# zcash/halo2

Measured on NVIDIA H100. Metric: msm_pairs_per_s, higher is better.
Workload: dtype u32x8 (255-bit modular integers)

## Files before the change

### halo2_b200/csrc/capi_msm.cu

```cuda
#define H2_MSM_QUAD_ACCUM_REFS (g_ctx.small_accum_refs)
#include "util_kernels.cuh"
#include "msm.cuh"
#include "ipa.cuh"
#include "ntt.cuh"
#include "ecfft.cuh"
#include "fixedbase.cuh"

struct PassBases { const affine *bases; uint32_t c = 0, mode = 0; uint64_t stride = 0; };
static PassBases pass_bases(const BaseSet *b) {
    if (b->dtable.p) return {b->dtable.as<affine>(), H2_FB_BITS, 2, b->n};
    if (b->table.p) return {b->table.as<affine>(), b->c, 1, b->n};
    return {b->buf.as<affine>()};
}


static int exclusive_scan_u32(uint32_t *d, uint64_t n, cudaStream_t s, const uint32_t *only_if = nullptr) {
    const uint64_t per_block = (uint64_t)H2_SCAN_BLOCK * H2_SCAN_ITEMS;
    uint32_t nb = (uint32_t)((n + per_block - 1) / per_block);
    if (g_ctx.scan_blocks.ensure((size_t)nb * 4 + 16)) return 1;
    uint32_t *bs = g_ctx.scan_blocks.as<uint32_t>();
    LAUNCH(scan_block_sums_kernel, nb, H2_SCAN_BLOCK, 0, s, d, n, bs, only_if);
    LAUNCH(scan_single_block_kernel, 1, H2_SCAN_BLOCK, 0, s, bs, nb, only_if);
    LAUNCH(scan_apply_kernel, nb, H2_SCAN_BLOCK, 0, s, d, n, bs, only_if);
    return 0;
// ... 108 lines not shown
        return msm_issue_or_replay(issue, !bc, d_scalars, d_bases, d_out, n, stride, H2_FB_BITS, fp.sets, scalars_mont, out_canonical, fast, s);
    }
    const uint32_t glv = (!fixed && X.glv_on && n < (1ull << 30)) ? 1u : 0u;
    if (c == 0) c = X.window_override ? X.window_override : msm_default_window(n, glv);
    if (c > 24) return fail("msm: window bits > 24");
    const uint32_t K = (bc && !fixed && bc->k > 1) ? bc->k : 1u;
    const uint32_t force_cap = X.sort_bins ? 0u : H2_MSM_NO_BINS;
    MsmPlan p;
    msm_make_plan(p, n, c, 0, 0, fixed, stride, glv, sets, force_cap);
    p.chunks = K;
    p.fast = (fixed == 1 && !bc && fast && p.cap != 0) ? 1u : 0u;
    if (ran_fast) *ran_fast = p.fast != 0;
    if (p.fast && p.T < p.cap) { p.T = p.cap; p.acc_chunk[0] = p.T; }
    p.natural = (p.fast && p.G <= X.natural_max_buckets && p.max_refs <= 2 * H2_MSM_QUAD_ACCUM_REFS && (X.accum_ways <= 1 || X.accum_ways >= 12)) ? 1u : 0u;
    MsmPlan pk[H2_MAX_UPLOAD_CHUNKS];
    size_t first[H2_MAX_UPLOAD_CHUNKS + 1];
    for (uint32_t j = 0; j <= K; j++) first[j] = chunk_first(n, K, j);
    uint64_t ref_space = 0, max_items = 0, part_total = 0;
    uint32_t t_max = 0;
    for (uint32_t j = 0; j < K; j++) {
        if (K == 1) pk[0] = p;
        else msm_make_plan(pk[j], first[j + 1] - first[j], c, 0, 0, fixed, stride, glv, sets, force_cap);
        if (pk[j].ref_space >= (1ull << 32)) return fail("msm: n * windows exceeds 2^32 references");
        ref_space = pk[j].ref_space > ref_space ? pk[j].ref_space : ref_space;
        max_items = pk[j].max_items > max_items ? pk[j].max_items : max_items;
        part_total = pk[j].part_total > part_total ? pk[j].part_total : part_total;
        t_max = pk[j].T > t_max ? pk[j].T : t_max;
    }
    bool thread_per_item = false;
    for (uint32_t j = 0; j < K; j++) thread_per_item |= pk[j].max_refs > (pk[j].fixed ? 2 : 1) * H2_MSM_QUAD_ACCUM_REFS;
    record(fixed, c, p.W, p.sets, thread_per_item ? 1u : 0u, p.natural, p.fast);
    uint64_t ba_space = 0;
    if (!fixed && X.ba_rounds) {
        size_t free_b = 0, total_b = 0;
        CU(cudaMemGetInfo(&free_b, &total_b));
        for (uint32_t j = 0; j < K; j++) {
            if (pk[j].max_refs > H2_MSM_QUAD_ACCUM_REFS && (uint64_t)K * pk[j].ref_space * 56 <= free_b / 2) msm_plan_ba(pk[j], X.ba_rounds, X.ba_target);
            if (pk[j].ba) ba_space = pk[j].ref_space > ba_space ? pk[j].ref_space : ba_space;
        }
    }
    if (K == 1) p.ba = pk[0].ba;
    if (ba_space)
        for (uint32_t r = 0; r < H2_BA_MAX_ROUNDS; r++)
            if (X.ba_lv[r].ensure(K * ((ba_space >> (r + 1)) + 1) * sizeof(affine))) return 1;
    if (glv && (X.bases_phi.ensure(n * sizeof(affine)) || X.glv_parts.ensure(n * 32))) return 1;
    if (fixed && (uint64_t)p.W * stride >= (1ull << 31)) return fail("msm: window table too large for 31-bit references");
    if (p.G >= (1ull << 32) || n >= (1ull << 31)) return fail("msm: n * windows exceeds 2^32 references");
    if (scalars_mont && X.scal_canon.ensure(n * p.sets * sizeof(fe))) return 1;
    const size_t small_words = 2 * (t_max + 2) + 8;
    part_total += 1;
    if (X.counts.ensure(K * (p.G + 1) * 4) || X.cursor.ensure(K * 2 * p.G * 4) || X.refs.ensure(K * ref_space * 4) ||
        X.size_hist.ensure(K * small_words * 4) || X.items.ensure(K * max_items * sizeof(uint2)) ||
        X.bucket_sum.ensure(K * p.G * sizeof(xyzz)) || X.pkey.ensure(K * part_total * 4) || X.pstart.ensure(K * part_total * 4) ||
        X.pend.ensure(K * part_total * 4) || X.ppt.ensure(K * part_total * sizeof(xyzz)) ||
        X.ra_t.ensure((size_t)p.Wb * p.m1 * sizeof(xyzz)) || X.ra_e.ensure((size_t)p.Wb * p.m1 * sizeof(xyzz)) ||
        X.r0.ensure((size_t)p.Wb * p.nb0 * H2_R0_ROWS * sizeof(xyzz)) || X.r1.ensure((size_t)p.Wb * p.r1_rows * sizeof(xyzz)) ||
        X.wsum.ensure((size_t)p.Wb * sizeof(xyzz)))
        return 1;
    MsmBuffers Mk[H2_MAX_UPLOAD_CHUNKS];
    for (uint32_t j = 0; j < K; j++) {
        MsmBuffers &M = Mk[j];
        const size_t o = first[j];
        M.scalars = d_scalars + o; M.bases = d_bases + o; M.bases_phi = X.bases_phi.as<affine>() + o;
        M.glv_parts = X.glv_parts.as<uint32_t>() + 8 * o; M.scalars_mont = scalars_mont ? 1u : 0u;
        M.scal_canon = X.scal_canon.as<fe>() + o;
        M.counts = X.counts.as<uint32_t>() + j * (p.G + 1); M.cursor = X.cursor.as<uint32_t>() + j * 2 * p.G; M.cursor2 = M.cursor + p.G;
        M.refs = X.refs.as<uint32_t>() + j * ref_space;
        M.size_hist = X.size_hist.as<uint32_t>() + j * small_words; M.size_cursor = M.size_hist + (pk[j].T + 2); M.flags = M.size_cursor + (pk[j].T + 2);
        M.items = X.items.as<uint2>() + j * max_items;
        M.bucket_sum = X.bucket_sum.as<xyzz>() + j * p.G;
        for (uint32_t r = 0; r < H2_BA_MAX_ROUNDS; r++) M.ba[r] = ba_space ? X.ba_lv[r].as<affine>() + j * ((ba_space >> (r + 1)) + 1) : nullptr;
        M.pkey = X.pkey.as<uint32_t>() + j * part_total; M.pstart = X.pstart.as<uint32_t>() + j * part_total;
        M.pend = X.pend.as<uint32_t>() + j * part_total; M.ppt = X.ppt.as<xyzz>() + j * part_total;
        M.ra_t = X.ra_t.as<xyzz>(); M.ra_e = X.ra_e.as<xyzz>(); M.r0 = X.r0.as<xyzz>(); M.r1 = X.r1.as<xyzz>();
        M.wsum = X.wsum.as<xyzz>(); M.result = d_out;
    }
    X.last_flags = Mk[0].flags;

    {
        const uint64_t per_block = (uint64_t)H2_SCAN_BLOCK * H2_SCAN_ITEMS;
        if (X.scan_blocks.ensure((size_t)((p.G + 1 + per_block - 1) / per_block) * 4 + 16)) return 1;
    }
    issue = [&]() -> int {
        if (!p.fast) CU(cudaMemsetAsync(X.counts.p, 0, K * (p.G + 1) * 4, s));
        CU(cudaMemsetAsync(X.cursor.p, 0, K * 2 * p.G * 4, s));
        CU(cudaMemsetAsync(X.size_hist.p, 0, K * small_words * 4, s));
        CU(cudaMemsetAsync(X.bucket_sum.p, 0, K * p.G * sizeof(xyzz), s));
        if (!p.fast) CU(cudaMemsetAsync(X.pkey.p, 0xff, K * part_total * 4, s));

        auto k_bin = msm_bin_kernel<P, PS>;
        auto k_hist = msm_hist_kernel<P, PS>;
        auto k_scatter = msm_scatter_kernel<P, PS>;
        auto k_ihist = msm_item_hist_kernel<P, PS>;
        auto k_ibases = msm_item_bases_kernel<P, PS>;
        auto k_iplace = msm_item_place_kernel<P, PS>;
        auto k_accum0 = msm_accum0_kernel<P, PS>;
        auto k_accum0q = msm_accum0_quad_kernel<P, PS>;
        auto k_accum0p2 = msm_accum0_pair_kernel<P, PS>;
        auto k_accum0s2 = msm_accum0_split_kernel<P, PS, 2>;
        auto k_accum0s4 = msm_accum0_split_kernel<P, PS, 4>;
        auto k_accum0m2 = msm_accum0_multi_kernel<P, PS, 2>;
        auto k_accum0m4 = msm_accum0_multi_kernel<P, PS, 4>;
        auto k_ba = X.ba_variant == 1 ? msm_ba_round_kernel<P, PS, 4, 5> : X.ba_variant == 2 ? msm_ba_round_kernel<P, PS, 2, 4>
                  : X.ba_variant == 3 ? msm_ba_round_kernel<P, PS, 2, 5> : msm_ba_round_kernel<P, PS, 4, 4>;
        auto k_accum0p = msm_accum0_pts_kernel<P, PS>;
        auto k_accumN = msm_accumN_kernel<P, PS>;
        auto k_rest = msm_accum_rest_kernel<P, PS>;
        auto k_reduceA = msm_reduceA_kernel<P, PS>;
        auto k_r0 = msm_r0_kernel<P, PS>;
        auto k_r1 = msm_r1_kernel<P, PS>;
        auto k_wsum = msm_wsum_kernel<P, PS>;
        auto k_final = msm_final_kernel<P, PS>;
        for (uint32_t j = 0; j < K; j++) {
            const MsmPlan &q = pk[j];
            const MsmBuffers &M = Mk[j];
            if (bc && bc->k) {
                for (uint32_t e = (K > 1 ? j : 0); e < (K > 1 ? j + 1 : bc->k); e++) {
                    if (bc->wait_recorded(2 * e + 1)) return fail("msm: the upload of the inputs failed");
                    CU(cudaStreamWaitEvent(s, bc->ev_scal[e], 0));
                }
            }
            if (q.cap == 0) CU(cudaMemsetAsync(M.flags + 1, 0x01, 4, s));
            else LAUNCH(k_bin, blocks_for(q.n * q.sets, 256), 256, 0, s, q, M);
            if (!q.fast) {
                LAUNCH(k_hist, blocks_for(q.n * q.sets, 256), 256, 0, s, q, M);
                if (exclusive_scan_u32(M.counts, q.G + 1, s, M.flags + 1)) return 1;
                LAUNCH(k_scatter, blocks_for(q.n * q.sets, 256), 256, 0, s, q, M);
            }
            if (!q.natural) {
                LAUNCH(k_ihist, blocks_for(q.G, 256), 256, 0, s, q, M);
                LAUNCH(k_ibases, 1, 32, 0, s, q, M);
                LAUNCH(k_iplace, blocks_for(q.G, 256), 256, 0, s, q, M);
            }
            if (bc && bc->k) {
                for (uint32_t e = (K > 1 ? j : 0); e < (K > 1 ? j + 1 : bc->k); e++) {
                    if (bc->wait_recorded(2 * e + 2)) return fail("msm: the upload of the inputs failed");
                    CU(cudaStreamWaitEvent(s, bc->ev[e], 0));
                }
            }
            if (q.glv) {
                auto k_phi = msm_phi_kernel<P, PS>;
                LAUNCH(k_phi, blocks_for(q.n, 256), 256, 0, s, M.bases, M.bases_phi, (uint64_t)q.n);
            }
            prof_begin(PROF_MSM_ACCUM0, s);
            if (q.max_refs <= (q.fixed ? 2 : 1) * H2_MSM_QUAD_ACCUM_REFS) {
                if (X.accum_ways == 4) LAUNCH(k_accum0m4, blocks_for(q.max_items * 16, 128), 128, 0, s, q, M);
                else if (X.accum_ways == 2) LAUNCH(k_accum0m2, blocks_for(q.max_items * 8, 128), 128, 0, s, q, M);
                else if (X.accum_ways == 0) LAUNCH(k_accum0p2, blocks_for(q.max_items * 2, 128), 128, 0, s, q, M);
                else if (X.accum_ways == 12) LAUNCH(k_accum0s2, blocks_for(q.max_items * 2, 128), 128, 0, s, q, M);
                else if (X.accum_ways == 14) LAUNCH(k_accum0s4, blocks_for(q.max_items * 4, 128), 128, 0, s, q, M);
                else LAUNCH(k_accum0q, blocks_for(q.max_items * 4, 128), 128, 0, s, q, M);
            }
            else {
                for (uint32_t r = 1; r <= q.ba; r++)
                    LAUNCH(k_ba, blocks_for((q.max_items + q.ba_m[r - 1] - 1) / q.ba_m[r - 1], 128), 128, 0, s, q, M, r);
                if (q.ba) LAUNCH(k_accum0p, blocks_for(q.max_items, 128), 128, 0, s, q, M);
                LAUNCH(k_accum0, blocks_for(q.max_items, 128), 128, 0, s, q, M);
            }
            prof_end(s);
            if (!q.fast) {
                if (q.acc_levels > 1) LAUNCH(k_accumN, blocks_for(q.acc_threads[1], 128), 128, 0, s, q, M, 1u);
                if (q.acc_levels > 2) LAUNCH(k_accumN, blocks_for(q.acc_threads[2], 128), 128, 0, s, q, M, 2u);
                if (q.acc_levels > 3) LAUNCH(k_rest, 1, 256, 0, s, q, M);
            }
        }
        const MsmBuffers &M = Mk[0];
        LAUNCH(k_reduceA, blocks_for((uint64_t)p.Wb * p.m1 * 4, 128), 128, 0, s, p, M);
        LAUNCH(k_r0, blocks_for((uint64_t)p.Wb * p.nb0 * (2 + p.bits0) * 4, 128), 128, 0, s, p, M);
        LAUNCH(k_r1, p.Wb * p.r1_rows, 4 * H2_R1_QUADS, 0, s, p, M);
        LAUNCH(k_wsum, p.Wb, 128, 0, s, p, M);
        LAUNCH(k_final, 1, 64, 0, s, p, M, (uint32_t)out_canonical);
        return 0;
    };
    return msm_issue_or_replay(issue, fixed && !bc, d_scalars, d_bases, d_out, n, stride, c, sets, scalars_mont, out_canonical, fast, s);
}

static int msm_dispatch(int curve, const fe *d_scalars, int scalars_mont, const PassBases &B, size_t n, jacobian *d_out, int out_canonical,
                        cudaStream_t s, const BasesChunks *bc, uint32_t sets, bool fast = false, bool rerun = false, bool *ran_fast = nullptr) {
    return by_curve(curve, [&](auto p, auto ps) {
        return msm_run<decltype(p), decltype(ps)>(d_scalars, scalars_mont, B.bases, n, B.c, B.mode, B.stride, d_out, out_canonical, s, bc, sets,
                                                  fast, rerun, ran_fast);
    });
}

struct PassOut { void *host; bool affine = false; void *peer = nullptr; int peer_dev = -1; };
static int msm_pass(int curve, const fe *d_scalars, int scalars_mont, const PassBases &B, size_t n, uint32_t sets, jacobian *d_result,
                    int canon, const PassOut &to, const BasesChunks *bc = nullptr, const std::function<int(int)> &issued = nullptr) {
    Context &X = g_ctx;
    cudaStream_t s = X.stream;
    if (to.affine && X.ec_out.ensure(sets * sizeof(affine))) return 1;
    for (int attempt = 0; attempt < 2; attempt++) {
        bool fast = false;
        int rc = msm_dispatch(curve, d_scalars, scalars_mont, B, n, d_result, to.affine ? 0 : canon, s, bc, sets,
                              attempt == 0 && B.mode == 1 && X.fast_on && !bc, attempt == 1, &fast);
        if (issued) rc = issued(rc);
        if (rc) return rc;
        if (to.affine) {
            const uint32_t nb = blocks_for((sets + H2_NORM_CHUNK - 1) / H2_NORM_CHUNK, 64);
            auto normalize = [&](auto p, auto) {
                LAUNCH(normalize_kernel<decltype(p)>, nb, 64, 0, s, (const xyzz *)nullptr, d_result, 0, X.ec_out.as<affine>(), canon, (uint64_t)sets);
                return 0;
            };
            if (by_curve(curve, normalize)) return 1;
            CU(cudaMemcpyAsync(to.host, X.ec_out.p, sets * sizeof(affine), cudaMemcpyDeviceToHost, s));
        } else if (to.peer) {
            CU(cudaMemcpyPeerAsync(to.peer, to.peer_dev, d_result, X.device, sets * sizeof(jacobian), s));
        } else {
            CU(cudaMemcpyAsync(to.host, d_result, sets * sizeof(jacobian), cudaMemcpyDeviceToHost, s));
        }
        if (fast) {
            if (!X.h_flags) CU(cudaHostAlloc((void **)&X.h_flags, 2 * sizeof(uint32_t), cudaHostAllocDefault));
            CU(cudaMemcpyAsync(X.h_flags, X.last_flags, 2 * sizeof(uint32_t), cudaMemcpyDeviceToHost, s));
        }
        CU(cudaStreamSynchronize(s));
        if (!fast || (X.h_flags[0] == 0 && X.h_flags[1] == 0)) break;
    }
    return 0;
}
static uint32_t table_window(size_t n) {
    uint32_t lg = 0;
    while ((1ull << (lg + 1)) <= n) lg++;
    uint32_t want = lg + 2;
    if (want <= 9) return 8;
    if (want <= 15) return 15;
    if (want == 16) return 15;
    if (want <= 18) return 16;
    if (want <= 20) return 17;
    return 20;
}
static int build_table(BaseSet *b, uint32_t c, cudaStream_t s) {
    if (c == 0) c = table_window(b->n);
    if (c < 4 || c > 24) return fail("window table: window bits must be in [4, 24]");
    uint32_t W = (256 + c - 1) / c;
    if ((uint64_t)W * b->n >= (1ull << 31)) return fail("window table: too many points");
    if (b->table.ensure((size_t)W * b->n * sizeof(affine))) return 1;
    if (by_curve(b->curve, [&](auto p, auto ps) {
            auto k = msm_table_kernel<decltype(p), decltype(ps)>;
            LAUNCH(k, blocks_for(b->n, 128), 128, 0, s, b->buf.as<affine>(), b->table.as<affine>(), (uint64_t)b->n, (uint64_t)b->n, c, W);
            return 0;
        }))
        return 1;
    b->c = c; b->W = W;
    return 0;
}
#define H2_FB_MAX_POINTS ((1u << 15) + 2u)
static int build_direct(BaseSet *b, cudaStream_t s) {
    if (b->n > H2_FB_MAX_POINTS) return fail("H2_BASES_DIRECT: at most 2^15 + 2 points (256 KiB of table per point)");
    if (b->c != H2_FB_BITS || b->W != H2_FB_WINDOWS) return fail("H2_BASES_DIRECT: needs the 8-bit window table");
    if (b->dtable.ensure((size_t)H2_FB_WINDOWS * H2_FB_MULTIPLES * b->n * sizeof(affine))) return 1;
    const uint64_t threads = (uint64_t)H2_FB_WINDOWS * b->n;
    return by_curve(b->curve, [&](auto p, auto ps) {
        auto k = fb_table_kernel<decltype(p), decltype(ps)>;
        LAUNCH(k, blocks_for(threads, 128), 128, 0, s, (const affine *)b->table.as<affine>(), b->dtable.as<affine>(), (uint64_t)b->n, (uint64_t)b->n);
        return 0;
// ... 541 lines not shown
```

### halo2_b200/csrc/ctx.cuh

```cuda
#pragma once
#include <cuda_runtime.h>

#include <atomic>
#include <condition_variable>
#include <cstdio>
#include <cstdlib>
#include <cstring>
#include <functional>
#include <map>
#include <mutex>
#include <string>
#include <thread>
#include <vector>

#include "../../include/halo2_b200.h"
#define H2_MAX_UPLOAD_CHUNKS 4
#define H2_MAX_DEVICES 16
#include "curve.cuh"

using namespace h2;

int fail(const std::string &m);
const std::string &last_error_string();
#define CU(expr)                                                                                         \
// ... 73 lines not shown
    bool ready = false;
    int device = -1;
    cudaStream_t stream = nullptr;
    cudaStream_t copy_stream = nullptr;
    cudaEvent_t ev_scalars_up = nullptr, ev_bases_up[H2_MAX_UPLOAD_CHUNKS] = {}, ev_scal_up[H2_MAX_UPLOAD_CHUNKS] = {};
    uint32_t chunk_min_log = 19;
    cudaEvent_t ev_splice = nullptr;
    uint32_t window_override = 0;
    const uint32_t *last_flags = nullptr;
    uint32_t fast_on = 1;
    uint64_t natural_max_buckets = 1ull << 14;
    uint32_t last_plan[8] = {};
    bool have_plan = false;
    uint32_t *h_flags = nullptr;
    uint32_t sort_bins = 1;
    uint32_t glv_on = 1;
    uint32_t accum_ways = 12;
    uint32_t poly_cta = 0;
    uint64_t small_accum_refs = 1ull << 20;
    uint32_t ntt_tma = 0;
    uint32_t ba_variant = 3;
    uint32_t ba_rounds = 0, ba_target = 32;
    uint32_t ecfft_quad = 1;
    DevBuf scal_in, bases_in, bases_phi, glv_parts, scal_canon, counts, cursor, refs, size_hist, items, bucket_sum, pkey, pstart, pend, ppt, ra_t, ra_e, r0, r1,
        wsum, scan_blocks, result, misc, ba_lv[3];
    DevBuf ntt_io, ntt_out, ntt_work, pow2;
    DevBuf col_tab;
    DevBuf ec_work, ec_io, ec_out;
    DevBuf fb_a, fb_b;
    DevBuf multi_parts;
    StageRing stage;
    DevBuf ast_code, ast_consts;
    DevBuf po_lvl, po_q, po_pts;
    DevBuf lk_keys, lk_u32;
    DevBuf kg_tab, kg_map;
    DevBuf as_edge, as_cell, as_slot;
    DevBuf gp_val, gp_aux;
    std::vector<TwiddleEntry *> twiddles;
    uint64_t tw_stamp = 0;
    std::map<uint64_t, BaseSet *> shards;
    std::map<uint64_t, IpaSession *> ipa;
    std::map<uint64_t, PolyBuf *> polys;
    std::vector<MsmGraph> graphs;
    uint64_t graph_stamp = 0;
    uint32_t graphs_on = 1;
    std::vector<PolyBuf *> poly_pool;
    size_t poly_pool_bytes = 0;
    std::vector<IpaSession *> ipa_pool;
};
#define H2_MAX_LANES 16
extern Context g_ctxs[H2_MAX_DEVICES];
extern Context g_lanes[H2_MAX_LANES];
extern Context *g_primary;
extern thread_local Context *g_cur;
extern thread_local uint64_t g_cur_epoch;
extern std::atomic<uint64_t> g_epoch;
extern Context g_dead;
static inline Context &cur_ctx() {
    if (!g_cur) return *g_primary;
    if (g_cur_epoch != g_epoch.load(std::memory_order_relaxed)) return g_dead;
    return *g_cur;
}
static inline void set_cur(Context *c) { g_cur = c; g_cur_epoch = g_epoch.load(); }
#define g_ctx (cur_ctx())
extern std::mutex g_life_mu, g_reg_mu;
struct CtxLock {
    std::lock_guard<std::mutex> g;
    CtxLock() : g(cur_ctx().mu.m) {}
};
uint64_t new_handle();
bool on_lane();
extern std::map<uint64_t, BaseSet *> g_bases;
struct BasesRef {
    BaseSet *b = nullptr;
    explicit BasesRef(uint64_t handle, bool open_session = false);
    ~BasesRef();
    BasesRef(const BasesRef &) = delete;
    BasesRef &operator=(const BasesRef &) = delete;
};
void bases_session_end(uint64_t handle);
struct ProfSpan { int kind; cudaEvent_t e0, e1; };
extern std::atomic<bool> g_prof_on;
extern std::vector<ProfSpan> g_prof;
enum { PROF_MSM_ACCUM0 = 0, PROF_NTT_PASS = 1, PROF_KINDS = 2 };
void prof_begin(int kind, cudaStream_t s);
void prof_end(cudaStream_t s);
extern std::atomic<uint64_t> g_launches;

#define LAUNCH(kernel, grid, block, smem, stream, ...)                                                   \
    do {                                                                                                 \
        kernel<<<(grid), (block), (smem), (stream)>>>(__VA_ARGS__);                                      \
        g_launches.fetch_add(1, std::memory_order_relaxed);                                              \
        cudaError_t e_ = cudaGetLastError();                                                             \
        if (e_ != cudaSuccess) return fail(std::string(#kernel) + " launch: " + cudaGetErrorString(e_)); \
    } while (0)

int upload_async(void *d_dst, const void *h_src, size_t bytes, cudaStream_t s);
int download_sync(void *h_dst, const void *d_src, size_t bytes, cudaStream_t s);
void h2_set_staging(int on);
int require_ready();
struct StreamSplice {
    explicit StreamSplice(cudaStream_t s);
    ~StreamSplice();
    StreamSplice(const StreamSplice &) = delete;
    StreamSplice &operator=(const StreamSplice &) = delete;
    Context &X;
    cudaStream_t s;
    int failed = 0;
};
static inline uint32_t blocks_for(uint64_t n, uint32_t bs) { return (uint32_t)((n + bs - 1) / bs); }

struct HostArgs {
    struct Need { const void *p; const char *name; bool required = true; };
    HostArgs(const char *who, int repr) : who(who), repr(repr) {}
    int check(std::initializer_list<Need> needs = {}) const;
    bool canon() const { return repr == H2_REPR_CANONICAL; }
    bool mont() const { return repr == H2_REPR_MONTGOMERY; }
    template <class P> fe elem(const void *bytes) const {
        fe x;
        memcpy(x.v, bytes, 32);
        return mont() ? x : fe_to_mont<P>(x);
    }
    int up(int field, fe *d, const void *h, size_t n, cudaStream_t s) const;
    int to_mont(int field, fe *d, size_t n, cudaStream_t s) const;
    int from_mont(int field, fe *d, size_t n, cudaStream_t s) const;
    int down(int field, void *h, const fe *d, size_t n, cudaStream_t s) const;
    const char *who;
    int repr;
};
extern std::map<uint64_t, PolyBuf *> g_shared_polys;
struct PolyArgs {
    explicit PolyArgs(const char *who, int field = -1) : who(who), field(field), field_given(field >= 0) {}
    ~PolyArgs();
    PolyBuf *out(uint64_t h, const char *name, uint64_t off, uint64_t len, const char *len_name) { return find(true, h, name, -1, off, len, len_name); }
    PolyBuf *in(uint64_t h, const char *name, uint64_t off, uint64_t len, const char *len_name) { return find(false, h, name, -1, off, len, len_name); }
    PolyBuf *out(uint64_t h, const char *name, uint64_t len, const char *len_name) { return out(h, name, 0, len, len_name); }
    PolyBuf *in(uint64_t h, const char *name, uint64_t len, const char *len_name) { return in(h, name, 0, len, len_name); }
    using Polys = std::vector<PolyBuf *>;
    int out(const uint64_t *h, size_t n, const char *name, uint64_t off, uint64_t len, const char *len_name, Polys &v) { return find(true, h, n, name, off, len, len_name, v); }
    int out(const uint64_t *h, size_t n, const char *name, uint64_t len, const char *len_name, Polys &v) { return find(true, h, n, name, 0, len, len_name, v); }
    int in(const uint64_t *h, size_t n, const char *name, uint64_t len, const char *len_name, Polys &v) { return find(false, h, n, name, 0, len, len_name, v); }
    int distinct(const char *in_place_out = nullptr, const char *in_place_in = nullptr);
    PolyArgs(const PolyArgs &) = delete;
    PolyArgs &operator=(const PolyArgs &) = delete;

  private:
    struct Arg { PolyBuf *p; bool out; const char *name; int64_t i; };
    std::string who;
    int field;
    bool field_given;
    std::vector<Arg> args;
    std::vector<PolyBuf *> held;
    PolyBuf *find(bool out, uint64_t h, const char *name, int64_t i, uint64_t off, uint64_t len, const char *len_name);
    int find(bool out, const uint64_t *h, size_t n, const char *name, uint64_t off, uint64_t len, const char *len_name, Polys &v);
};
struct ColTable {
    fe *const *cols;
    fe *data;
};
int col_table(const std::vector<PolyBuf *> &cols, const void *data, size_t bytes, cudaStream_t s, ColTable *t);
int shared_poly_free(uint64_t h);
template <class F> static int by_field(int field, F &&f) {
    if (field == H2_FIELD_FP) return f(FpParams{});
    if (field == H2_FIELD_FQ) return f(FqParams{});
    return fail("unknown field id");
}
template <class F> static int by_curve(int curve, F &&f) {
// ... 24 lines not shown
```

### halo2_b200/csrc/msm.cuh

```cuda
#pragma once
#include "curve.cuh"
#include "glv.cuh"

namespace h2 {

H2_HD affine ld_affine(const affine *p) { affine r; r.x = fe_load(&p->x); r.y = fe_load(&p->y); return r; }
H2_HD void st_affine(affine *p, const affine &a) { fe_store(&p->x, a.x); fe_store(&p->y, a.y); }
H2_HD xyzz ld_xyzz(const xyzz *p) { xyzz r; r.x = fe_load(&p->x); r.y = fe_load(&p->y); r.zz = fe_load(&p->zz); r.zzz = fe_load(&p->zzz); return r; }
H2_HD void st_xyzz(xyzz *p, const xyzz &a) { fe_store(&p->x, a.x); fe_store(&p->y, a.y); fe_store(&p->zz, a.zz); fe_store(&p->zzz, a.zzz); }
H2_HD void st_jacobian(jacobian *p, const jacobian &a) { fe_store(&p->x, a.x); fe_store(&p->y, a.y); fe_store(&p->z, a.z); }

#define H2_MSM_INVALID_KEY 0xffffffffu
#define H2_MSM_MAX_LEVELS 12
#define H2_R0_LOG 3
#define H2_R0_ROWS 5

struct MsmPlan {
    uint64_t n;
    uint32_t c;
    uint32_t glv;
    uint32_t chunks;
    uint32_t cap;
    uint32_t cap_top;
    uint64_t g_top;
// ... 615 lines not shown
    for (uint32_t e = 0; e < halves; e++) {
        uint32_t carry = 0;
        for (uint32_t w0 = 0; w0 < p.W; w0 += 4) {
            uint32_t slot[4], gid[4], ref[4];
            bool act[4];
#pragma unroll
            for (int k = 0; k < 4; k++) {
                uint32_t w = w0 + k;
                int32_t d = w < p.W ? Msm<P, PS>::next_digit(part[e], w, p.c, carry) : 0;
                act[k] = in && d != 0;
                uint32_t mag = d < 0 ? (uint32_t)(-d) : (uint32_t)d;
                gid[k] = (uint32_t)((uint64_t)(p.fixed ? set : (w < p.W ? w : 0)) * p.B + (act[k] ? mag - 1 : 0));
                ref[k] = ((uint32_t)idx + (uint32_t)(p.fixed && w < p.W ? (uint64_t)w * p.stride : 0)) | (e << 30) |
                         ((((uint32_t)(d < 0)) ^ sneg[e]) << 31);
                slot[k] = warp_inc<true>(M.cursor + gid[k], act[k]);
            }
#pragma unroll
            for (int k = 0; k < 4; k++)
                if (act[k]) {
                    uint32_t lo, cap;
                    if (Msm<P, PS>::bin_of(p, gid[k], lo, cap) && slot[k] < cap) M.refs[lo + slot[k]] = ref[k];
                    else full = true;
                }
        }
    }
    if (full) M.flags[1] = 1;
}
template <class P, class PS> __global__ void __launch_bounds__(256) msm_hist_kernel(const MsmPlan p, const MsmBuffers M) {
    if (!M.flags[1]) return;
    uint64_t i = (uint64_t)blockIdx.x * blockDim.x + threadIdx.x;
    bool in = i < p.n * p.sets;
    const uint64_t set = p.fixed && in ? i / p.n : 0;
    uint32_t part[2][8] = {{0, 0, 0, 0, 0, 0, 0, 0}, {0, 0, 0, 0, 0, 0, 0, 0}}, sneg[2] = {0, 0};
    const uint32_t halves = p.glv ? 2u : 1u;
    if (in) Msm<P, PS>::load_parts(p, M, i, true, part, sneg);
    for (uint32_t e = 0; e < halves; e++) {
        uint32_t carry = 0;
        for (uint32_t w = 0; w < p.W; w++) {
            int32_t d = Msm<P, PS>::next_digit(part[e], w, p.c, carry);
            bool act = in && d != 0;
            uint32_t mag = d < 0 ? (uint32_t)(-d) : (uint32_t)d;
            uint64_t g = (uint64_t)(p.fixed ? set : w) * p.B + (act ? mag - 1 : 0);
            warp_inc<false>(M.counts + g, act);
        }
    }
}
template <class P, class PS> __global__ void __launch_bounds__(256) msm_scatter_kernel(const MsmPlan p, const MsmBuffers M) {
    if (!M.flags[1]) return;
    uint64_t i = (uint64_t)blockIdx.x * blockDim.x + threadIdx.x;
    bool in = i < p.n * p.sets;
    const uint64_t set = p.fixed && in ? i / p.n : 0, idx = p.fixed && in ? i % p.n : i;
    uint32_t part[2][8] = {{0, 0, 0, 0, 0, 0, 0, 0}, {0, 0, 0, 0, 0, 0, 0, 0}}, sneg[2] = {0, 0};
    const uint32_t halves = p.glv ? 2u : 1u;
    if (in) Msm<P, PS>::load_parts(p, M, i, false, part, sneg);
    for (uint32_t e = 0; e < halves; e++) {
        uint32_t carry = 0;
        for (uint32_t w0 = 0; w0 < p.W; w0 += 4) {
            uint32_t slot[4], gid[4], ref[4];
            bool act[4];
#pragma unroll
            for (int k = 0; k < 4; k++) {
                uint32_t w = w0 + k;
                int32_t d = w < p.W ? Msm<P, PS>::next_digit(part[e], w, p.c, carry) : 0;
                act[k] = in && d != 0;
                uint32_t mag = d < 0 ? (uint32_t)(-d) : (uint32_t)d;
                gid[k] = (uint32_t)((uint64_t)(p.fixed ? set : (w < p.W ? w : 0)) * p.B + (act[k] ? mag - 1 : 0));
                ref[k] = ((uint32_t)idx + (uint32_t)(p.fixed && w < p.W ? (uint64_t)w * p.stride : 0)) | (e << 30) |
                         ((((uint32_t)(d < 0)) ^ sneg[e]) << 31);
                slot[k] = warp_inc<true>(M.cursor2 + gid[k], act[k]);
            }
#pragma unroll
            for (int k = 0; k < 4; k++)
                if (act[k]) M.refs[M.counts[gid[k]] + slot[k]] = ref[k];
        }
    }
}
template <class P, class PS> __global__ void __launch_bounds__(256) msm_phi_kernel(const affine *bases, affine *out, uint64_t n) {
    uint64_t i = (uint64_t)blockIdx.x * blockDim.x + threadIdx.x;
    if (i >= n) return;
    affine b = ld_affine(bases + i);
    b.x = fe_mul<P>(b.x, glv_zeta<P>());
    st_affine(out + i, b);
}
template <class P, class PS> __global__ void __launch_bounds__(256) msm_item_hist_kernel(const MsmPlan p, const MsmBuffers M) {
    if (p.fast && M.flags[1]) return;
    uint64_t g = (uint64_t)blockIdx.x * blockDim.x + threadIdx.x;
    uint32_t nfull = 0, rem = 0;
    if (g < p.G) Msm<P, PS>::count_items(p, M, g, nfull, rem);
    if (nfull) atomicAdd(M.size_hist + p.T, nfull);
    warp_inc<false>(M.size_hist + rem, rem != 0);
}
template <class P, class PS> __global__ void msm_item_bases_kernel(const MsmPlan p, const MsmBuffers M) {
    if (threadIdx.x == 0 && blockIdx.x == 0) Msm<P, PS>::size_bases_body(p, M);
}
template <class P, class PS> __global__ void __launch_bounds__(256) msm_item_place_kernel(const MsmPlan p, const MsmBuffers M) {
    if (p.fast && M.flags[1]) return;
    uint64_t g = (uint64_t)blockIdx.x * blockDim.x + threadIdx.x;
    uint32_t nfull = 0, rem = 0, lo = 0;
    if (g < p.G) { Msm<P, PS>::count_items(p, M, g, nfull, rem); lo = Msm<P, PS>::bucket_lo(p, M, g); }
    if (nfull) {
        uint32_t at = atomicAdd(M.size_cursor + p.T, nfull);
        for (uint32_t k = 0; k < nfull; k++) M.items[at + k] = make_uint2((uint32_t)g, lo + k * p.T);
    }
    uint32_t at = warp_inc<true>(M.size_cursor + rem, rem != 0);
    if (rem) M.items[at] = make_uint2((uint32_t)g, lo + nfull * p.T);
}
template <class P, class PS> __global__ void __launch_bounds__(128) msm_table_kernel(const affine *bases, affine *table, uint64_t count, uint64_t stride,
                                                                                    uint32_t c, uint32_t W) {
    Msm<P, PS>::table_body(bases, table, count, stride, c, W, (uint64_t)blockIdx.x * blockDim.x + threadIdx.x);
}
template <class P, class PS> __global__ void __launch_bounds__(128, 5) msm_accum0_kernel(const MsmPlan p, const MsmBuffers M) {
    uint64_t t = (uint64_t)blockIdx.x * blockDim.x + threadIdx.x;
    Msm<P, PS>::accum0_body(p, M, t);
}
template <class P, class PS, int U, int MINB> __global__ void __launch_bounds__(128, MINB) msm_ba_round_kernel(const MsmPlan p, const MsmBuffers M, uint32_t r) {
    Msm<P, PS>::template ba_round_body<128, U>(p, M, r, (uint64_t)blockIdx.x * blockDim.x + threadIdx.x);
}
template <class P, class PS> __global__ void __launch_bounds__(128, 5) msm_accum0_pts_kernel(const MsmPlan p, const MsmBuffers M) {
    Msm<P, PS>::accum0_pts_body(p, M, (uint64_t)blockIdx.x * blockDim.x + threadIdx.x);
}
template <class P, class PS> __global__ void __launch_bounds__(128) msm_accum0_quad_kernel(const MsmPlan p, const MsmBuffers M) {
    uint64_t t = ((uint64_t)blockIdx.x * blockDim.x + threadIdx.x) >> 2;
    Msm<P, PS>::template accum0_body<QuadAdd, true>(p, M, t);
}
template <class P, class PS> __global__ void __launch_bounds__(128) msm_accum0_pair_kernel(const MsmPlan p, const MsmBuffers M) {
    uint64_t t = ((uint64_t)blockIdx.x * blockDim.x + threadIdx.x) >> 1;
    Msm<P, PS>::template accum0_body<PairAdd, true>(p, M, t);
}
template <class P, class PS, int WAYS> __global__ void __launch_bounds__(128) msm_accum0_multi_kernel(const MsmPlan p, const MsmBuffers M) {
    const uint64_t t = ((uint64_t)blockIdx.x * blockDim.x + threadIdx.x) / (4 * WAYS);
    if (p.fast && M.flags[1]) return;
    if (t >= M.size_hist[p.T + 1]) return;
    const uint32_t lane = threadIdx.x & 31u, h = (lane >> 2) & (WAYS - 1);
    const uint32_t gmask = (WAYS == 8 ? 0xffffffffu : ((1u << (4 * WAYS)) - 1u) << (lane & ~(4u * WAYS - 1u)));
    const uint2 it = M.items[t];
    const uint32_t g = it.x, start = it.y, lo = Msm<P, PS>::bucket_lo(p, M, g), hi = Msm<P, PS>::bucket_hi(p, M, g);
    const uint32_t end = start + p.T < hi ? start + p.T : hi;
    xyzz acc = xyzz_identity();
    for (uint32_t pos = start + h; pos < end; pos += WAYS) {
        const uint32_t ref = M.refs[pos];
        affine b;
        if (p.glv) b = ld_affine(((ref >> 30) & 1u ? M.bases_phi : M.bases) + (ref & 0x3fffffffu));
        else b = ld_affine(M.bases + (ref & 0x7fffffffu));
        if (ref >> 31) b.y = fe_neg<P>(b.y);
        xyzz_add_mixed_quad<P>(acc, b);
    }
#pragma unroll
    for (int step = WAYS / 2; step >= 1; step >>= 1) {
        xyzz other;
#pragma unroll
        for (int i = 0; i < 8; i++) {
            other.x.v[i] = __shfl_down_sync(gmask, acc.x.v[i], 4 * step, 4 * WAYS);
            other.y.v[i] = __shfl_down_sync(gmask, acc.y.v[i], 4 * step, 4 * WAYS);
            other.zz.v[i] = __shfl_down_sync(gmask, acc.zz.v[i], 4 * step, 4 * WAYS);
            other.zzz.v[i] = __shfl_down_sync(gmask, acc.zzz.v[i], 4 * step, 4 * WAYS);
        }
        if ((int)h < step) xyzz_add_quad<P>(acc, other);
    }
    if (h == 0) {
        typename Msm<P, PS>::Flusher F; F.M = &M; F.p = &p;
        F.flush(g, start, end, acc, p.part_offset[1] + Msm<P, PS>::item_slot(p, start, start == lo));
    }
}
template <class P, class PS, int WAYS> __global__ void __launch_bounds__(128) msm_accum0_split_kernel(const MsmPlan p, const MsmBuffers M) {
    const uint64_t t = ((uint64_t)blockIdx.x * blockDim.x + threadIdx.x) / WAYS;
    if (p.fast && M.flags[1]) return;
    const uint32_t lane = threadIdx.x & 31u, h = lane & (WAYS - 1);
    uint2 it;
    bool live = true;
    if (p.natural) {
        live = t < p.G;
        it = make_uint2((uint32_t)(live ? t : 0), live ? Msm<P, PS>::bucket_lo(p, M, live ? t : 0) : 0u);
    } else {
        live = t < M.size_hist[p.T + 1];
        it = live ? M.items[t] : make_uint2(0u, 0u);
    }
    const uint32_t g = it.x, start = it.y, lo = Msm<P, PS>::bucket_lo(p, M, g), hi = live ? Msm<P, PS>::bucket_hi(p, M, g) : start;
    const uint32_t end = start + p.T < hi ? start + p.T : hi;
    xyzz acc = xyzz_identity();
    if (start + h < end) {
        uint32_t ref = M.refs[start + h];
        affine nxt = Msm<P, PS>::ref_point(p, M, ref);
        for (uint32_t pos = start + h; pos < end; pos += WAYS) {
            affine b = nxt;
            const uint32_t neg = ref >> 31;
            if (pos + WAYS < end) { ref = M.refs[pos + WAYS]; nxt = Msm<P, PS>::ref_point(p, M, ref); }
            if (neg) b.y = fe_neg<P>(b.y);
            xyzz_add_mixed<P>(acc, b);
        }
    }
#pragma unroll
    for (int step = WAYS / 2; step >= 1; step >>= 1) {
        xyzz other;
#pragma unroll
        for (int i = 0; i < 8; i++) {
            other.x.v[i] = __shfl_down_sync(0xffffffffu, acc.x.v[i], step, WAYS);
            other.y.v[i] = __shfl_down_sync(0xffffffffu, acc.y.v[i], step, WAYS);
            other.zz.v[i] = __shfl_down_sync(0xffffffffu, acc.zz.v[i], step, WAYS);
            other.zzz.v[i] = __shfl_down_sync(0xffffffffu, acc.zzz.v[i], step, WAYS);
        }
        if ((int)h < step) xyzz_add<P>(acc, other);
    }
    if (h == 0 && live && end > start) {
        typename Msm<P, PS>::Flusher F; F.M = &M; F.p = &p;
        F.flush(g, start, end, acc, p.part_offset[1] + Msm<P, PS>::item_slot(p, start, start == lo));
    }
}
template <class P, class PS> __global__ void __launch_bounds__(128) msm_accumN_kernel(const MsmPlan p, const MsmBuffers M, uint32_t lv) {
    uint64_t t = (uint64_t)blockIdx.x * blockDim.x + threadIdx.x;
    if (t < p.acc_threads[lv]) Msm<P, PS>::accumN_body(p, M, lv, t);
}
template <class P, class PS> __global__ void __launch_bounds__(256) msm_accum_rest_kernel(const MsmPlan p, const MsmBuffers M) {
    if (!M.flags[0]) return;
    for (uint32_t lv = 3; lv < p.acc_levels; lv++) {
        for (uint64_t t = threadIdx.x; t < p.acc_threads[lv]; t += blockDim.x) Msm<P, PS>::accumN_body(p, M, lv, t);
        __threadfence();
        __syncthreads();
    }
}
template <class P, class PS> __global__ void __launch_bounds__(128) msm_reduceA_kernel(const MsmPlan p, const MsmBuffers M) {
    uint64_t t = ((uint64_t)blockIdx.x * blockDim.x + threadIdx.x) >> 2;
    Msm<P, PS>::template reduceA_body<QuadAdd>(p, M, t);
}

template <class P> __device__ __forceinline__ void block_tree_sum(xyzz *sh, xyzz &v, uint32_t row, uint32_t lane, uint32_t width) {
    st_xyzz(sh + row * width + lane, v);
    __syncthreads();
    for (uint32_t off = width >> 1; off > 0; off >>= 1) {
        if (lane < off) {
            xyzz o = ld_xyzz(sh + row * width + lane + off);
            xyzz_add<P>(v, o);
            st_xyzz(sh + row * width + lane, v);
        }
        __syncthreads();
    }
}
template <class P> __device__ __forceinline__ void quad_tree_sum(xyzz *sh, xyzz &v, uint32_t qd, uint32_t quads) {
    st_xyzz(sh + qd, v);
    __syncthreads();
    for (uint32_t off = quads >> 1; off > 0; off >>= 1) {
        if (qd < off) {
            xyzz o = ld_xyzz(sh + qd + off);
            xyzz_add_quad<P>(v, o);
            st_xyzz(sh + qd, v);
        }
        __syncthreads();
    }
}
template <class P, class PS> __global__ void __launch_bounds__(128) msm_r0_kernel(const MsmPlan p, const MsmBuffers M) {
    uint64_t tid = ((uint64_t)blockIdx.x * blockDim.x + threadIdx.x) >> 2;
    const uint32_t rows = 2 + p.bits0;
    if (tid >= (uint64_t)p.Wb * p.nb0 * rows) return;
    uint32_t row = (uint32_t)(tid % rows);
    uint64_t wb = tid / rows;
    uint32_t w = (uint32_t)(wb / p.nb0), blk = (uint32_t)(wb % p.nb0);
    xyzz v = xyzz_identity();
    const uint32_t want = row >= 2 ? 1u << (row - 2) : 0u;
    auto next_lane = [&](uint32_t l) { while (l < (1u << H2_R0_LOG) && (l & want) != want) l++; return l; };
    uint32_t lane = next_lane(0);
    xyzz nxt = lane < (1u << H2_R0_LOG) ? Msm<P, PS>::r0_contrib(p, M, w, blk, row, lane) : xyzz_identity();
    while (lane < (1u << H2_R0_LOG)) {
        const xyzz c = nxt;
        lane = next_lane(lane + 1);
        if (lane < (1u << H2_R0_LOG)) nxt = Msm<P, PS>::r0_contrib(p, M, w, blk, row, lane);
        xyzz_add_quad<P>(v, c);
    }
    st_xyzz(M.r0 + ((uint64_t)w * p.nb0 + blk) * H2_R0_ROWS + row, v);
}
#define H2_R1_QUADS 128
template <class P, class PS> __global__ void __launch_bounds__(4 * H2_R1_QUADS) msm_r1_kernel(const MsmPlan p, const MsmBuffers M) {
    __shared__ xyzz sh[H2_R1_QUADS];
    const uint32_t w = blockIdx.x / p.r1_rows, row = blockIdx.x % p.r1_rows, qd = threadIdx.x >> 2;
    xyzz v = xyzz_identity();
    xyzz nxt = qd < p.nb0 ? Msm<P, PS>::r1_contrib(p, M, w, row, qd) : xyzz_identity();
    for (uint32_t blk = qd; blk < p.nb0; blk += H2_R1_QUADS) {
        const xyzz c = nxt;
        if (blk + H2_R1_QUADS < p.nb0) nxt = Msm<P, PS>::r1_contrib(p, M, w, row, blk + H2_R1_QUADS);
        xyzz_add_quad<P>(v, c);
    }
    quad_tree_sum<P>(sh, v, qd, H2_R1_QUADS);
    if (threadIdx.x == 0) st_xyzz(M.r1 + (uint64_t)w * p.r1_rows + row, v);
}
template <class P, class PS> __global__ void __launch_bounds__(128) msm_wsum_kernel(const MsmPlan p, const MsmBuffers M) {
    __shared__ xyzz sh[32];
    const uint32_t w = blockIdx.x, r = threadIdx.x >> 2;
    xyzz v = xyzz_identity();
    if (r < p.r1_rows) {
        v = ld_xyzz(M.r1 + (uint64_t)w * p.r1_rows + r);
        uint32_t shift = (p.fixed ? 0 : p.c * w) + (r >= 2 ? (r - 2) + p.l0 : 0);
        xyzz_shift_quad<P>(v, shift);
    }
    quad_tree_sum<P>(sh, v, r, 32);
    if (threadIdx.x == 0) st_xyzz(M.wsum + w, v);
}
template <class P, class PS> __global__ void __launch_bounds__(64) msm_final_kernel(const MsmPlan p, const MsmBuffers M, uint32_t out_canonical) {
    __shared__ xyzz sh[16];
    if (p.fixed) {
        for (uint32_t set = threadIdx.x; set < p.sets; set += 64) Msm<P, PS>::finish(M, ld_xyzz(M.wsum + set), out_canonical, set);
        return;
    }
    const uint32_t qd = threadIdx.x >> 2;
    xyzz v = xyzz_identity();
    for (uint32_t w = qd; w < p.Wb; w += 16) { xyzz c = ld_xyzz(M.wsum + w); xyzz_add_quad<P>(v, c); }
    quad_tree_sum<P>(sh, v, qd, 16);
    if (threadIdx.x == 0) Msm<P, PS>::finish(M, v, out_canonical);
}
// ... 69 lines not shown
```

Baseline: 242.3 million.

## Aggregate item-size histogram atomics in shared memory and add serial reduceA path

Measured after the change: 249.7 million (median of 6 runs). 1.03x the previous value.

```diff
diff --git a/halo2_b200/csrc/capi_msm.cu b/halo2_b200/csrc/capi_msm.cu
--- a/halo2_b200/csrc/capi_msm.cu
+++ b/halo2_b200/csrc/capi_msm.cu
@@ -214,11 +214,13 @@
         if (X.scan_blocks.ensure((size_t)((p.G + 1 + per_block - 1) / per_block) * 4 + 16)) return 1;
     }
     issue = [&]() -> int {
+        prof_begin(PROF_MSM_SORT, s);
         if (!p.fast) CU(cudaMemsetAsync(X.counts.p, 0, K * (p.G + 1) * 4, s));
         CU(cudaMemsetAsync(X.cursor.p, 0, K * 2 * p.G * 4, s));
         CU(cudaMemsetAsync(X.size_hist.p, 0, K * small_words * 4, s));
         CU(cudaMemsetAsync(X.bucket_sum.p, 0, K * p.G * sizeof(xyzz), s));
         if (!p.fast) CU(cudaMemsetAsync(X.pkey.p, 0xff, K * part_total * 4, s));
+        prof_end(s);
 
         auto k_bin = msm_bin_kernel<P, PS>;
         auto k_hist = msm_hist_kernel<P, PS>;
@@ -239,6 +241,7 @@
         auto k_accumN = msm_accumN_kernel<P, PS>;
         auto k_rest = msm_accum_rest_kernel<P, PS>;
         auto k_reduceA = msm_reduceA_kernel<P, PS>;
+        auto k_reduceA1 = msm_reduceA_serial_kernel<P, PS>;
         auto k_r0 = msm_r0_kernel<P, PS>;
         auto k_r1 = msm_r1_kernel<P, PS>;
         auto k_wsum = msm_wsum_kernel<P, PS>;
@@ -252,6 +255,7 @@
                     CU(cudaStreamWaitEvent(s, bc->ev_scal[e], 0));
                 }
             }
+            prof_begin(PROF_MSM_SORT, s);
             if (q.cap == 0) CU(cudaMemsetAsync(M.flags + 1, 0x01, 4, s));
             else LAUNCH(k_bin, blocks_for(q.n * q.sets, 256), 256, 0, s, q, M);
             if (!q.fast) {
@@ -259,10 +263,13 @@
                 if (exclusive_scan_u32(M.counts, q.G + 1, s, M.flags + 1)) return 1;
                 LAUNCH(k_scatter, blocks_for(q.n * q.sets, 256), 256, 0, s, q, M);
             }
+            prof_end(s);
             if (!q.natural) {
+                prof_begin(PROF_MSM_ITEMS, s);
                 LAUNCH(k_ihist, blocks_for(q.G, 256), 256, 0, s, q, M);
                 LAUNCH(k_ibases, 1, 32, 0, s, q, M);
                 LAUNCH(k_iplace, blocks_for(q.G, 256), 256, 0, s, q, M);
+                prof_end(s);
             }
             if (bc && bc->k) {
                 for (uint32_t e = (K > 1 ? j : 0); e < (K > 1 ? j + 1 : bc->k); e++) {
@@ -272,7 +279,9 @@
             }
             if (q.glv) {
                 auto k_phi = msm_phi_kernel<P, PS>;
+                prof_begin(PROF_MSM_PHI, s);
                 LAUNCH(k_phi, blocks_for(q.n, 256), 256, 0, s, M.bases, M.bases_phi, (uint64_t)q.n);
+                prof_end(s);
             }
             prof_begin(PROF_MSM_ACCUM0, s);
             if (q.max_refs <= (q.fixed ? 2 : 1) * H2_MSM_QUAD_ACCUM_REFS) {
@@ -291,17 +300,22 @@
             }
             prof_end(s);
             if (!q.fast) {
+                prof_begin(PROF_MSM_MERGE, s);
                 if (q.acc_levels > 1) LAUNCH(k_accumN, blocks_for(q.acc_threads[1], 128), 128, 0, s, q, M, 1u);
                 if (q.acc_levels > 2) LAUNCH(k_accumN, blocks_for(q.acc_threads[2], 128), 128, 0, s, q, M, 2u);
                 if (q.acc_levels > 3) LAUNCH(k_rest, 1, 256, 0, s, q, M);
+                prof_end(s);
             }
         }
         const MsmBuffers &M = Mk[0];
-        LAUNCH(k_reduceA, blocks_for((uint64_t)p.Wb * p.m1 * 4, 128), 128, 0, s, p, M);
+        prof_begin(PROF_MSM_TAIL, s);
+        if (!p.fixed && p.G > (1ull << 17)) LAUNCH(k_reduceA1, blocks_for((uint64_t)p.Wb * p.m1, 128), 128, 0, s, p, M);
+        else LAUNCH(k_reduceA, blocks_for((uint64_t)p.Wb * p.m1 * 4, 128), 128, 0, s, p, M);
         LAUNCH(k_r0, blocks_for((uint64_t)p.Wb * p.nb0 * (2 + p.bits0) * 4, 128), 128, 0, s, p, M);
         LAUNCH(k_r1, p.Wb * p.r1_rows, 4 * H2_R1_QUADS, 0, s, p, M);
         LAUNCH(k_wsum, p.Wb, 128, 0, s, p, M);
         LAUNCH(k_final, 1, 64, 0, s, p, M, (uint32_t)out_canonical);
+        prof_end(s);
         return 0;
     };
     return msm_issue_or_replay(issue, fixed && !bc, d_scalars, d_bases, d_out, n, stride, c, sets, scalars_mont, out_canonical, fast, s);
diff --git a/halo2_b200/csrc/ctx.cuh b/halo2_b200/csrc/ctx.cuh
--- a/halo2_b200/csrc/ctx.cuh
+++ b/halo2_b200/csrc/ctx.cuh
@@ -179,7 +179,8 @@
 struct ProfSpan { int kind; cudaEvent_t e0, e1; };
 extern std::atomic<bool> g_prof_on;
 extern std::vector<ProfSpan> g_prof;
-enum { PROF_MSM_ACCUM0 = 0, PROF_NTT_PASS = 1, PROF_KINDS = 2 };
+enum { PROF_MSM_ACCUM0 = 0, PROF_NTT_PASS = 1, PROF_MSM_SORT = 2, PROF_MSM_ITEMS = 3, PROF_MSM_PHI = 4, PROF_MSM_MERGE = 5,
+       PROF_MSM_TAIL = 6, PROF_KINDS = 7 };
 void prof_begin(int kind, cudaStream_t s);
 void prof_end(cudaStream_t s);
 extern std::atomic<uint64_t> g_launches;
diff --git a/halo2_b200/csrc/msm.cuh b/halo2_b200/csrc/msm.cuh
--- a/halo2_b200/csrc/msm.cuh
+++ b/halo2_b200/csrc/msm.cuh
@@ -721,28 +721,44 @@
     b.x = fe_mul<P>(b.x, glv_zeta<P>());
     st_affine(out + i, b);
 }
+#define H2_ITEM_SH 512
 template <class P, class PS> __global__ void __launch_bounds__(256) msm_item_hist_kernel(const MsmPlan p, const MsmBuffers M) {
+    __shared__ uint32_t hist[H2_ITEM_SH];
     if (p.fast && M.flags[1]) return;
+    for (uint32_t i = threadIdx.x; i < H2_ITEM_SH; i += blockDim.x) hist[i] = 0;
+    __syncthreads();
     uint64_t g = (uint64_t)blockIdx.x * blockDim.x + threadIdx.x;
     uint32_t nfull = 0, rem = 0;
     if (g < p.G) Msm<P, PS>::count_items(p, M, g, nfull, rem);
-    if (nfull) atomicAdd(M.size_hist + p.T, nfull);
-    warp_inc<false>(M.size_hist + rem, rem != 0);
+    if (nfull) atomicAdd(p.T < H2_ITEM_SH ? hist + p.T : M.size_hist + p.T, nfull);
+    if (rem) atomicAdd(rem < H2_ITEM_SH ? hist + rem : M.size_hist + rem, 1u);
+    __syncthreads();
+    for (uint32_t i = threadIdx.x; i < H2_ITEM_SH; i += blockDim.x)
+        if (hist[i]) atomicAdd(M.size_hist + i, hist[i]);
 }
 template <class P, class PS> __global__ void msm_item_bases_kernel(const MsmPlan p, const MsmBuffers M) {
     if (threadIdx.x == 0 && blockIdx.x == 0) Msm<P, PS>::size_bases_body(p, M);
 }
 template <class P, class PS> __global__ void __launch_bounds__(256) msm_item_place_kernel(const MsmPlan p, const MsmBuffers M) {
+    __shared__ uint32_t cnt[H2_ITEM_SH];
     if (p.fast && M.flags[1]) return;
+    for (uint32_t i = threadIdx.x; i < H2_ITEM_SH; i += blockDim.x) cnt[i] = 0;
+    __syncthreads();
     uint64_t g = (uint64_t)blockIdx.x * blockDim.x + threadIdx.x;
-    uint32_t nfull = 0, rem = 0, lo = 0;
+    uint32_t nfull = 0, rem = 0, lo = 0, at_full = 0, at_rem = 0;
     if (g < p.G) { Msm<P, PS>::count_items(p, M, g, nfull, rem); lo = Msm<P, PS>::bucket_lo(p, M, g); }
+    const bool sh_full = p.T < H2_ITEM_SH, sh_rem = rem < H2_ITEM_SH;
+    if (nfull) at_full = sh_full ? atomicAdd(cnt + p.T, nfull) : atomicAdd(M.size_cursor + p.T, nfull);
+    if (rem) at_rem = sh_rem ? atomicAdd(cnt + rem, 1u) : atomicAdd(M.size_cursor + rem, 1u);
+    __syncthreads();
+    for (uint32_t i = threadIdx.x; i < H2_ITEM_SH; i += blockDim.x)
+        if (cnt[i]) cnt[i] = atomicAdd(M.size_cursor + i, cnt[i]);
+    __syncthreads();
     if (nfull) {
-        uint32_t at = atomicAdd(M.size_cursor + p.T, nfull);
+        const uint32_t at = at_full + (sh_full ? cnt[p.T] : 0u);
         for (uint32_t k = 0; k < nfull; k++) M.items[at + k] = make_uint2((uint32_t)g, lo + k * p.T);
     }
-    uint32_t at = warp_inc<true>(M.size_cursor + rem, rem != 0);
-    if (rem) M.items[at] = make_uint2((uint32_t)g, lo + nfull * p.T);
+    if (rem) M.items[at_rem + (sh_rem ? cnt[rem] : 0u)] = make_uint2((uint32_t)g, lo + nfull * p.T);
 }
 template <class P, class PS> __global__ void __launch_bounds__(128) msm_table_kernel(const affine *bases, affine *table, uint64_t count, uint64_t stride,
                                                                                     uint32_t c, uint32_t W) {
@@ -861,6 +877,9 @@
     uint64_t t = ((uint64_t)blockIdx.x * blockDim.x + threadIdx.x) >> 2;
     Msm<P, PS>::template reduceA_body<QuadAdd>(p, M, t);
 }
+template <class P, class PS> __global__ void __launch_bounds__(128) msm_reduceA_serial_kernel(const MsmPlan p, const MsmBuffers M) {
+    Msm<P, PS>::template reduceA_body<SerialAdd>(p, M, (uint64_t)blockIdx.x * blockDim.x + threadIdx.x);
+}
 
 template <class P> __device__ __forceinline__ void block_tree_sum(xyzz *sh, xyzz &v, uint32_t row, uint32_t lane, uint32_t width) {
     st_xyzz(sh + row * width + lane, v);
```
